# Huguet57/LIMO-Velo

Measured on AMD Instinct MI355X. Metric: KF-update iters/sec, 64k-pt scan vs 1M-pt map, higher is better.
Workload: dtype f32 (kNN/plane fit) + f64 (Jacobian rows, H^T H, 23-dof solve)

## Files before the change

### limo-velo_amd/csrc/lv_api.hip

```cpp
#include <cmath>
#include <cstdlib>
#include <cstring>
#include <limits>
#include <new>

#include "lv_filter.hpp"
#include "lv_host.hpp"
#include "lv_rebuild.hpp"
#include "lv_visibility.hpp"
#include "lv_paint.hpp"
#include "lv_place.hpp"

#include <chrono>

namespace lv {

static thread_local char g_err[512] = "";

void set_error(const char* fmt, ...) {
    va_list ap;
    va_start(ap, fmt);
    vsnprintf(g_err, sizeof(g_err), fmt, ap);
    va_end(ap);
}
// ... 43 lines not shown
    int grid = 1;
    bool fold_direct = false;
    bool tile_lpt = true;
    float4* d_qrec = nullptr;
    uint32_t qstride = 0;
    double* d_cpart[2] = {nullptr, nullptr};
    RankExchange ranks;
    uint32_t* d_wgcost[2] = {nullptr, nullptr};
    int pass_max_wg = 256;
    bool fused_pass = true;
    bool record_dump = false;
    bool last_update_fused = false;
    long long* d_pclk = nullptr;
    int pclk_wg = 0;
    bool keeper_by_cost = true;
    int fused_multi_round = -1;
    bool fused_ext = true;

    bool capture = false;
    size_t cap_n = 0;
    DebugOut dbg{};
    bool dbg_valid = false;
    bool qrec_valid = false;

    bool begin_pending = false;
    BeginArg h_begin;
    int fallback_base = 0;
    long mailbox_resyncs = 0;

    int pass_index = -1;
    bool coll_timed = false;
    bool fast_fit = false;
    bool multi_overlap = true;
    bool in_update = false;
    bool want_log = false;
    int passes_issued = 0;

    bool profiling = false;
    bool phase_clocks = false;
    long long* d_clk = nullptr;
    hipEvent_t ev_begin = nullptr, ev_end = nullptr;
    std::vector<hipEvent_t> ev_pass;
    hipEvent_t ev_mid = nullptr;
    std::vector<hipEvent_t> ev_coll;
    lv_timing timing{};
};

namespace {

struct SlowCall {
    const char* name;
    std::chrono::steady_clock::time_point t0;
    static double limit_ms() { static const double v = [] { const char* e = getenv("LV_SLOW_CALL_MS"); return e ? atof(e) : 0.0; }(); return v; }
    explicit SlowCall(const char* n) : name(n) { if (limit_ms() > 0.0) t0 = std::chrono::steady_clock::now(); }
    ~SlowCall() {
        if (limit_ms() > 0.0) {
            const double ms = std::chrono::duration<double, std::milli>(std::chrono::steady_clock::now() - t0).count();
            if (ms > limit_ms()) fprintf(stderr, "[limovelo_hip] slow call: %s took %.3f ms\n", name, ms);
        }
    }
};
#define LV_CHECK_CTX(ctx)                        \
    SlowCall _slow_call(__func__);               \
    do {                                         \
        if (!(ctx)) {                            \
            set_error("null context");           \
// ... 80 lines not shown
                const double theta = (A[q][q] - A[p][p]) / (2.0 * apq);
                const double t = (theta >= 0.0 ? 1.0 : -1.0) / (std::fabs(theta) + std::sqrt(theta * theta + 1.0));
                const double c = 1.0 / std::sqrt(t * t + 1.0), s = t * c;
                for (int k = 0; k < 6; ++k) {
                    const double akp = A[k][p], akq = A[k][q];
                    A[k][p] = c * akp - s * akq;
                    A[k][q] = s * akp + c * akq;
                }
                for (int k = 0; k < 6; ++k) {
                    const double apk = A[p][k], aqk = A[q][k];
                    A[p][k] = c * apk - s * aqk;
                    A[q][k] = s * apk + c * aqk;
                }
            }
    for (int i = 0; i < 6; ++i) eig[i] = A[i][i];
}

void unpack_sums(const double* rec, lv_sums* out) {
    int idx = 0;
    for (int i = 0; i < 12; ++i)
        for (int j = i; j < 12; ++j) {
            out->HTH[i * 12 + j] = rec[idx];
            out->HTH[j * 12 + i] = rec[idx];
            ++idx;
        }
    for (int i = 0; i < 12; ++i) out->HTh[i] = rec[78 + i];
    out->n_valid = (int64_t)rec[90];
    out->sum_h2 = rec[91];
}

int begin_device(lv_ctx* c, const double* x_host, bool defer, const ResidentFilter::Prior& prior = {}) {
    if (int rf = c->filter.begin_update(c->stream, c->d_kf, prior.dev != nullptr)) return rf;
    c->begin_pending = false;
    if (c->capture) LV_HIP(hipMemsetAsync(c->d_kf->level_hist, 0, sizeof(int) * 8, c->stream));
    if (defer && x_host && c->scan.n > 0 && c->map.view.m > 0) {
        std::memcpy(c->h_begin.x, x_host, sizeof(c->h_begin.x));
        std::memcpy(c->h_begin.P, x_host + NX, sizeof(c->h_begin.P));
        compute_pose_consts(c->h_begin.x, &c->h_begin.pose);
        c->begin_pending = true;
    } else {
        int rc = launch_kf_begin(c->stream, c->d_kf, c->d_io, x_host, prior.dev, prior.dev_in_kf);
        if (rc) return rc;
    }
    c->grid = fit_grid_size(c->scan.n, c->max_blocks);
    if ((uint32_t)c->scan.n > c->qstride) {
        uint32_t cap = c->qstride ? c->qstride : 4096;
        while (cap < (uint32_t)c->scan.n) cap *= 2;
        LV_HIP(hipStreamSynchronize(c->stream));
        hipFree(c->d_qrec);
        c->d_qrec = nullptr;
        c->qstride = 0;
        LV_HIP(hipMalloc(&c->d_qrec, (size_t)cap * qrec_slots(c->prm.NUM_MATCH_POINTS) * sizeof(float4)));
        c->qstride = cap;
    }
    return LV_OK;
}

int begin_common(lv_ctx* c, const lv_state* x, const double* P, bool defer = true) {
    KfHostIO* io = c->h_io;
    std::memcpy(io->x_in, x, sizeof(double) * NX);
    if (P) {
        std::memcpy(io->P_in, P, sizeof(double) * NS * NS);
    } else {
        for (int i = 0; i < NS * NS; ++i) io->P_in[i] = (i / NS == i % NS) ? 1.0 : 0.0;
    }
    c->update_seq = (c->update_seq + 1) & 0x3fffffff;
    return begin_device(c, io->x_in, defer);
// ... 92 lines not shown
    if (c->ranks.multi_rank() && !c->ranks.fits((size_t)nwg * partial_width(c))) return false;
    return c->fused_pass && !c->capture && !c->phase_clocks && c->prm.degeneracy_mode <= 1 && c->prm.NUM_MATCH_POINTS == KNN &&
           c->prm.lanes_per_query == 8 && (c->prm.estimate_extrinsics == 0 || c->fused_ext) && c->map.view.m > 0;
}

int update_fused(lv_ctx* c) {
    const int npass = c->prm.MAX_NUM_ITERS + 1;
    PassLaunch pl{};
    pl.map = &c->map.view;
    pl.scan = c->scan.d_sorted;
    pl.tile_order = (c->tile_lpt && c->scan.tile_points == 32u && c->scan.n_tiles == (c->scan.n + 31u) / 32u) ? c->scan.d_tile_order : nullptr;
    pl.n = c->scan.n;
    pl.kf = c->d_kf;
    pl.io = c->d_io;
    pl.sums_out = c->d_sums;
    pl.mp.R_inv = 1.0 / c->prm.LiDAR_noise;
    pl.mp.max_dist_plane_sq = c->prm.MAX_DIST_PLANE * c->prm.MAX_DIST_PLANE;
    pl.mp.planes_threshold = c->prm.PLANES_THRESHOLD;
    pl.mp.estimate_extrinsics = c->prm.estimate_extrinsics;
    pl.mp.fast_fit = c->fast_fit && !c->prm.estimate_extrinsics;
    pl.sp.R = c->prm.LiDAR_noise;
    pl.sp.R_inv = 1.0 / c->prm.LiDAR_noise;
    for (int i = 0; i < NS; ++i) pl.sp.limits[i] = c->prm.LIMITS[i];
    pl.sp.maximum_iter = c->prm.MAX_NUM_ITERS;
    pl.sp.estimate_extrinsics = c->prm.estimate_extrinsics;
    pl.sp.seq = c->update_seq;
    pl.sp.degeneracy_mode = 0;
    pl.sp.degeneracy_threshold = c->prm.degeneracy_threshold;
    int nwg = 0, rounds = 0, steps = 0, dedicated = 0;
    pass_grid_size(pass_geometry_points(c), c->pass_max_wg, &nwg, &steps, &rounds, &dedicated);
    const bool gathered = c->ranks.multi_rank();
    const size_t slot = (size_t)nwg * partial_width(c);
    pl.multi_overlap = c->multi_overlap;
    pl.qrec = c->record_dump ? c->d_qrec : nullptr;
    c->pclk_wg = nwg + dedicated;
    pl.qstride = c->qstride;
    c->qrec_valid = c->record_dump;
    c->last_update_fused = true;
    for (int i = 0; i <= npass; ++i) {
        const bool closing = i == npass;
        pl.mode = i == 0 ? (c->begin_pending ? 0 : 2) : 1;
        pl.recs_in = gathered ? c->ranks.d_gather[(i + 1) & 1] : c->d_cpart[(i + 1) & 1];
        pl.part_out = gathered ? c->ranks.part_out(i & 1, slot) : c->d_cpart[i & 1];
        pl.nrec = c->ranks.nrec(nwg);
        pl.cost_in = (i > 0 && c->keeper_by_cost) ? c->d_wgcost[(i + 1) & 1] : nullptr;
        pl.cost_out = c->d_wgcost[i & 1];
        pl.nwg = nwg;
        pl.rounds = closing ? 0 : rounds;
        pl.steps = steps;
        pl.dedicated = dedicated;
        pl.launch = i;
        pl.clk = c->d_pclk ? c->d_pclk + (size_t)i * (c->pass_max_wg + 1) * pass_clock_words() : nullptr;
        if (c->profiling && !closing) LV_HIP(hipEventRecord(c->ev_pass[3 * i + 0], c->stream));
        int rc = launch_pass(c->stream, pl, (i == 0 && c->begin_pending) ? &c->h_begin : nullptr);
        c->begin_pending = false;
        if (rc) return rc;
        if (c->profiling && !closing) LV_HIP(hipEventRecord(c->ev_pass[3 * i + 1], c->stream));
        if (gathered && !closing) {
            if (c->profiling) LV_HIP(hipEventRecord(c->ev_coll[2 * i], c->stream));
            if ((rc = c->ranks.exchange(c->stream, i, slot))) return rc;
            if (c->profiling) LV_HIP(hipEventRecord(c->ev_coll[2 * i + 1], c->stream));
        }
        if (c->profiling && !closing) LV_HIP(hipEventRecord(c->ev_pass[3 * i + 2], c->stream));
    }
    c->coll_timed = gathered && c->profiling;
    return LV_OK;
}

}

extern "C" {

void lv_default_params(lv_params* p) {
    if (!p) return;
    std::memset(p, 0, sizeof(*p));
    p->MAX_NUM_ITERS = 3;
    p->NUM_MATCH_POINTS = 5;
    p->MAX_DIST_PLANE = 2.0;
    p->PLANES_THRESHOLD = 5.e-2f;
// ... 31 lines not shown
        if (!warned) {
            warned = true;
            fprintf(stderr, "limovelo_hip: degeneracy_threshold = %g is set but has no effect: the degeneracy stage of the fork's "
                            "update_iterated_dyn_share_modified is not part of the reference mount; degeneracy_mode = 2 enables a "
                            "documented restatement, degeneracy_mode = 1 reports the eigenvalues (include/limovelo_hip.h)\n",
                    params->degeneracy_threshold);
        }
    }
    int ndev = 0;
    hipError_t e = hipGetDeviceCount(&ndev);
    if (e != hipSuccess || ndev <= 0) { set_error("no HIP device available (%s)", hipGetErrorString(e)); return LV_ENODEV; }
    if (device < 0 || device >= ndev) { set_error("device %d out of range (%d devices)", device, ndev); return LV_EINVAL; }
    LV_HIP(hipSetDevice(device));
    lv_ctx* c = new (std::nothrow) lv_ctx();
    if (!c) { set_error("out of host memory"); return LV_EINVAL; }
    c->prm = *params;
    c->device = device;
    c->scan.tile_points = 256u / (uint32_t)S;
    c->map.cell = params->voxel_size;
    hipDeviceProp_t prop;
    LV_HIP(hipGetDeviceProperties(&prop, device));
    int per_cu = 4;
    if (const char* e = getenv("LV_BLOCKS_PER_CU")) per_cu = atoi(e) > 0 ? atoi(e) : 4;
    if (const char* e = getenv("LV_TILE_LPT")) c->tile_lpt = atoi(e) != 0;
    if (const char* e = getenv("LV_SPIN_WAIT")) c->spin_wait = atoi(e) != 0;
    if (const char* e = getenv("LV_FUSED_PASS")) c->fused_pass = atoi(e) != 0;
    if (const char* e = getenv("LV_FUSED_EXT")) c->fused_ext = atoi(e) != 0;
    if (const char* e = getenv("LV_FUSED_MULTI")) c->fused_multi_round = atoi(e) != 0 ? 1 : 0;
    if (const char* e = getenv("LV_ASYNC_RELINEARISE")) c->rebuild.opt.async = atoi(e) != 0;
    if (const char* e = getenv("LV_RELIN_SLICE_WGS")) c->rebuild.opt.slice_wgs = (uint32_t)atol(e);
    if (const char* e = getenv("LV_RELIN_PAUSE_US")) c->rebuild.opt.pause_us = (uint32_t)atol(e);
    if (const char* e = getenv("LV_MULTI_OVERLAP")) c->multi_overlap = atoi(e) != 0;
    if (const char* e = getenv("LV_KEEPER_BY_COST")) c->keeper_by_cost = atoi(e) != 0;
    if (const char* e = getenv("LV_COMM_FUSED")) c->ranks.fused = atoi(e) != 0;
    if (const char* e = getenv("LV_SMALL_WINDOW")) c->scan.small_enabled = atoi(e) != 0;
    if (const char* e = getenv("LV_LARGE_WINDOW")) c->scan.large_enabled = atoi(e) != 0;
    if (const char* e = getenv("LV_MAIL_FILTER")) c->filter.mail_filter = atoi(e) != 0;
    if (const char* e = getenv("LV_SMALL_INSERT")) c->map.small_front = atoi(e) != 0;
    if (const char* e = getenv("LV_SURV_LIST")) c->map.surv_list = atoi(e) != 0;
    c->pass_max_wg = prop.multiProcessorCount;
    if (const char* e = getenv("LV_PASS_WG")) c->pass_max_wg = atoi(e) > 0 ? atoi(e) : c->pass_max_wg;
    if (const char* e = getenv("LV_PASS_CLK")) {
        if (atoi(e) != 0) {
            const size_t words = (size_t)(MAX_PASSES + 1) * (c->pass_max_wg + 1) * pass_clock_words();
            LV_HIP(hipMalloc(&c->d_pclk, words * sizeof(long long)));
            LV_HIP(hipMemset(c->d_pclk, 0, words * sizeof(long long)));
        }
    }
    c->max_blocks = prop.multiProcessorCount * per_cu;
    if (c->max_blocks < 64) c->max_blocks = 64;
    LV_HIP(hipStreamCreateWithFlags(&c->own_stream, hipStreamNonBlocking));
    c->stream = c->own_stream;
    LV_HIP(hipStreamCreateWithFlags(&c->side_stream, hipStreamNonBlocking));
    c->rebuild.create_streams(device, true);
    LV_HIP(hipEventCreateWithFlags(&c->ev_staged, hipEventDisableTiming));
    if (const char* e = getenv("LV_OVERLAP_INSERT")) c->overlap_insert = atoi(e) != 0;
    if (const char* e = getenv("LV_BATCH_PREDICT")) c->filter.batch_predict = atoi(e) != 0;
    if (const char* e = getenv("LV_MERGED_INSERT")) c->map.merged_back = atoi(e) != 0;
    if (const char* e = getenv("LV_SWEEP_EVICT")) c->map.sweep_evict = atoi(e) != 0;
    LV_HIP(hipMalloc(&c->d_kf, sizeof(KfDev)));
    LV_HIP(hipMemset(c->d_kf, 0, sizeof(KfDev)));
    if (int rf = c->filter.alloc()) return rf;
    LV_HIP(hipHostMalloc((void**)&c->h_kf, sizeof(KfDev), hipHostMallocDefault));
    std::memset(c->h_kf, 0, sizeof(KfDev));
    LV_HIP(hipHostMalloc((void**)&c->h_io, sizeof(KfHostIO), hipHostMallocMapped));
    std::memset(c->h_io, 0, sizeof(KfHostIO));
// ... 981 lines not shown
}

int lv_last_update_fused(lv_ctx* c) { return (c && c->last_update_fused) ? 1 : 0; }
int lv_last_passes(lv_ctx* c) { return c ? c->h_io->passes : 0; }

int lv_pass_geometry(size_t n_scan, int n_cus, int out[4]) {
    if (!out || n_cus < 1 || n_scan > 0xFFFFFFF0ull) { set_error("lv_pass_geometry: bad arguments"); return LV_EINVAL; }
    pass_grid_size((uint32_t)n_scan, n_cus, &out[0], &out[1], &out[2], &out[3]);
    return LV_OK;
}

int lv_set_fused_pass(lv_ctx* c, int enabled) {
    LV_CHECK_CTX(c);
    c->fused_pass = enabled != 0;
    return LV_OK;
}

int lv_set_option(lv_ctx* c, const char* name, int value) {
    LV_CHECK_CTX(c);
    if (!name) { set_error("null argument"); return LV_EINVAL; }
    if (c->in_update) { set_error("lv_set_option inside an update"); return LV_ESTATE; }
    const bool on = value != 0;
    if (!std::strcmp(name, "fused_pass")) c->fused_pass = on;
    else if (!std::strcmp(name, "fused_ext")) c->fused_ext = on;
    else if (!std::strcmp(name, "fast_fit")) c->fast_fit = on;
    else if (!std::strcmp(name, "async_relinearise")) c->rebuild.opt.async = on;
    else if (!std::strcmp(name, "async_relinearise_min")) c->rebuild.opt.async_min = value > 0 ? (size_t)value : 0;
    else if (!std::strcmp(name, "async_relinearise_pause_us")) c->rebuild.opt.pause_us = value > 0 ? (uint32_t)value : 0u;
    else if (!std::strcmp(name, "async_relinearise_slice_wgs")) c->rebuild.opt.slice_wgs = value > 0 ? (uint32_t)value : 0u;
    else if (!std::strcmp(name, "async_relinearise_journal_max")) c->rebuild.opt.journal_max = value > 0 ? (size_t)value : 1;
    else if (!std::strcmp(name, "async_relinearise_test_delay_ms")) c->rebuild.opt.test_delay_ms = value;
    else if (!std::strcmp(name, "async_relinearise_test_race")) c->rebuild.opt.test_race = on;
    else if (!std::strcmp(name, "multi_overlap")) c->multi_overlap = on;
    else if (!std::strcmp(name, "fused_multi_round")) c->fused_multi_round = on ? 1 : 0;
    else if (!std::strcmp(name, "keeper_by_cost")) c->keeper_by_cost = on;
    else if (!std::strcmp(name, "tile_lpt")) c->tile_lpt = on;
    else if (!std::strcmp(name, "spin_wait")) c->spin_wait = on;
    else if (!std::strcmp(name, "comm_fused")) c->ranks.fused = on;
    else if (!std::strcmp(name, "mail_filter")) c->filter.mail_filter = on;
    else if (!std::strcmp(name, "overlap_insert")) c->overlap_insert = on;
    else if (!std::strcmp(name, "batch_predict")) { if (int rp = c->filter.flush(c->stream, c->d_kf)) return rp; c->filter.batch_predict = on; }
    else if (!std::strcmp(name, "merged_insert")) c->map.merged_back = on;
    else if (!std::strcmp(name, "sweep_evict")) c->map.sweep_evict = on;
    else if (!std::strcmp(name, "small_window")) c->scan.small_enabled = on;
    else if (!std::strcmp(name, "large_window")) c->scan.large_enabled = on;
    else if (!std::strcmp(name, "small_insert")) c->map.small_front = on;
    else if (!std::strcmp(name, "survivor_list")) c->map.surv_list = on;
    else if (!std::strcmp(name, "batch_chunk_hypotheses")) c->batch.chunk_hyp = value > 0 ? value : 0;
    else { set_error("lv_set_option: unknown option '%s'", name); return LV_EINVAL; }
    return LV_OK;
}

int lv_get_pass_clocks(lv_ctx* c, long long* out, int capacity_wg, int* n_wg) {
    LV_CHECK_CTX(c);
    if (!c->d_pclk) { set_error("no pass clocks: create the context with LV_PASS_CLK=1 in the environment"); return LV_ESTATE; }
    const int slots = c->pass_max_wg + 1;
    if (!out) {
        if (n_wg) *n_wg = slots;
        return LV_OK;
    }
    if (capacity_wg < slots) { set_error("lv_get_pass_clocks: capacity %d < %d workgroup slots per launch", capacity_wg, slots); return LV_EINVAL; }
    LV_HIP(hipStreamSynchronize(c->stream));
    LV_HIP(hipMemcpy(out, c->d_pclk, (size_t)(c->prm.MAX_NUM_ITERS + 2) * slots * pass_clock_words() * sizeof(long long), hipMemcpyDeviceToHost));
    if (n_wg) *n_wg = c->pclk_wg;
    return LV_OK;
}
// ... 463 lines not shown
```

### limo-velo_amd/csrc/lv_host.hpp

```cpp
#pragma once
#include "lv_note.hpp"

#include <cstdarg>
#include <cstdio>
#include <vector>

#include "../../include/limovelo_hip.h"
#include "lv_device.hpp"
#include "lv_common.hpp"
#include "lv_exchange.hpp"
#include "lv_mapinc.hpp"

namespace lv {

struct MapStats {
    uint64_t living, ids, capacity;
    uint64_t pool_used[4], pool_cap[4];
    uint64_t slots_used[4], slots_cap[4];
    uint64_t tombstones, dropped;
    uint64_t relinearisations, incremental_adds;
    uint64_t bytes;
};

struct MapStore {
// ... 188 lines not shown
int launch_kf_begin(hipStream_t stream, KfDev* kf, KfHostIO* io, const double* x_host, const FilterDev* filt = nullptr, int filt_in_kf = 0);
int launch_reduce_groups(hipStream_t stream, const double* partials, int nblocks, double* groups, int* ngroups_out, KfDev* kf);
int solve_direct_records();
int launch_reduce_final(hipStream_t stream, const double* groups, int ngroups, double* sums, KfDev* kf);
struct SolveParams {
    double R;
    double R_inv;
    double limits[NS];
    int maximum_iter;
    int estimate_extrinsics;
    int seq;
    int degeneracy_mode;
    double degeneracy_threshold;
};
int launch_solve(hipStream_t stream, KfDev* kf, KfHostIO* io, const double* recs, int nrec, double* sums_out, const SolveParams& prm);
struct PassLaunch {
    const MapView* map;
    const float4* scan;
    const uint32_t* tile_order;
    uint32_t n;
    KfDev* kf;
    KfHostIO* io;
    const double* recs_in;
    double* part_out;
    double* sums_out;
    float4* qrec;
    long long* clk;
    uint32_t qstride;
    int nrec;
    int mode;
    int rounds, launch, nwg;
    const uint32_t* cost_in;
    uint32_t* cost_out;
    bool multi_overlap = true;
    int steps, dedicated;
    MatchParams mp;
    SolveParams sp;
};
void pass_grid_size(uint32_t n, int max_wg, int* nsearch, int* steps, int* rounds, int* dedicated);
constexpr int PK_DEFAULT_MAX_ROUNDS = 16;
int pass_clock_words();
int launch_pass(hipStream_t stream, const PassLaunch& pl, const BeginArg* begin);
int launch_filter_to_kf(hipStream_t stream, const FilterDev* f, KfDev* kf);
int launch_rows_from_matches(hipStream_t stream, const KfDev* kf, const float* p_world, const float* abcd, const float* dist,
                             uint32_t n, int estimate_extrinsics, double* H, double* h);
struct CloudPoint;
struct ScanStore {
    float4* d_raw = nullptr;
    float4* d_sorted = nullptr;
    uint32_t* d_keys = nullptr;
    uint32_t* d_keys_sorted = nullptr;
    uint32_t* d_idx = nullptr;
    uint32_t* d_idx_sorted = nullptr;
    void* d_sort_tmp = nullptr;
    size_t sort_tmp_bytes = 0;
    size_t capacity = 0;
    uint32_t n = 0;
    uint32_t* d_tile_order = nullptr;
    uint32_t n_tiles = 0, tile_cap = 0;
    uint32_t tile_points = 0;
    float4* d_in = nullptr;
    double* d_times = nullptr;
    float4* d_desk = nullptr;
    MotionState* d_states = nullptr;
    uint64_t* d_vkeys = nullptr;
    uint64_t* d_vkeys_sorted = nullptr;
    uint32_t* d_vidx = nullptr;
    uint32_t* d_vidx_sorted = nullptr;
    uint32_t* d_heads = nullptr;
    uint32_t* d_hpos = nullptr;
    unsigned* d_bounds = nullptr;
    void* d_vsort_tmp = nullptr;
    void* d_vscan_tmp = nullptr;
// ... 84 lines not shown
```

### limo-velo_amd/csrc/lv_match.hip

```cpp
#include "lv_host.hpp"
#include "lv_pass_dev.hpp"

#ifndef LV_HALF_CHUNK
#define LV_HALF_CHUNK 1
#endif
#ifndef LV_QR_SELECT
#define LV_QR_SELECT 1
#endif
#include "lv_search_dev.hpp"

namespace lv {

__device__ __forceinline__ void sort8(kkey (&c)[8]) {
    cswap(c[0], c[1]); cswap(c[2], c[3]); cswap(c[4], c[5]); cswap(c[6], c[7]);
    cswap(c[0], c[2]); cswap(c[1], c[3]); cswap(c[4], c[6]); cswap(c[5], c[7]);
    cswap(c[1], c[2]); cswap(c[5], c[6]);
    cswap(c[0], c[4]); cswap(c[1], c[5]); cswap(c[2], c[6]); cswap(c[3], c[7]);
    cswap(c[2], c[4]); cswap(c[3], c[5]);
    cswap(c[1], c[2]); cswap(c[3], c[4]); cswap(c[5], c[6]);
}
__device__ __forceinline__ void order_unimodal5(kkey (&c)[5]) {
    cswap(c[0], c[4]); cswap(c[1], c[3]); cswap(c[1], c[4]); cswap(c[2], c[4]); cswap(c[3], c[4]);
}
template <int K>
// ... 530 lines not shown
                if (lane == 0) atomicAdd(&kf->fallback_queries, 1);
                done = cells_attempt(map, ((wgeo.c0x >> 3) - 1) * 2, ((wgeo.c0y >> 3) - 1) * 2, ((wgeo.c0z >> 3) - 1) * 2, 6, search_radius(map, wgeo, 3),
                                     wx, wy, wz, lane, kw, s_pref, s_start);
                if (done) wbin = 3;
            }
        } else {
            float r = search_radius(map, wgeo, 2);
            int side = 3, bx = c2x - 1, by = c2y - 1, bz = c2z - 1;
            if (!(r > 0.f && (double)(r * r) >= max_dist_sq)) {
                side = 4;
                bx = c2x - 1 - ((wgeo.tx - (float)((c2x << 2) - CELL_OFFSET)) < 2.f ? 1 : 0);
                by = c2y - 1 - ((wgeo.ty - (float)((c2y << 2) - CELL_OFFSET)) < 2.f ? 1 : 0);
                bz = c2z - 1 - ((wgeo.tz - (float)((c2z << 2) - CELL_OFFSET)) < 2.f ? 1 : 0);
                r = block_radius(map, wgeo, 2, bx, by, bz, 4);
                if (lane == 0) atomicAdd(&kf->fallback_queries, 1);
            }
            done = cells_attempt(map, bx, by, bz, side, r, wx, wy, wz, lane, kw, s_pref, s_start, &wgeo, bound);
            if (done) wbin = side == 3 ? 2 : 3;
            stop = r > 0.f && (double)(r * r) >= max_dist_sq;
        }
        if (!done && !stop) { brute_attempt(map, wx, wy, wz, lane, kw); wbin = 4; }
    } else {
        if (lane == 0) atomicAdd(&kf->fallback_queries, 1);
        brute_attempt(map, wx, wy, wz, lane, kw);
        wbin = 4;
    }
    return wbin;
}

template <int S, bool DBG, int K>
__device__ __forceinline__ void knn_search(const MapView& map, KfDev* __restrict__ kf, float qx, float qy, float qz, int gl,
                                           kkey (&k)[K], uint32_t& bstart, int& src, long long* clk, bool hist,
                                           bool live, Xyz* stage0, double max_dist_sq, uint32_t* s_pref, uint32_t* s_start,
                                           bool* undecided = nullptr, uint32_t* bound_out = nullptr) {
    if (undecided) *undecided = false;
    if (map.m == 0) return;
    const QGeom geo = make_geom(map, qx, qy, qz);
    const bool finite = __builtin_isfinite(qx) && __builtin_isfinite(qy) && __builtin_isfinite(qz);
    const bool in_range = finite && geo.amax < CELL_FAR;
    bool decided = !live || !finite;
    int hist_bin = -1;
    uint32_t bound = 0x7FFFFFFFu;
    if (live && in_range) {
#pragma unroll
#ifndef LV_DIAG_LEVELS
#define LV_DIAG_LEVELS 2
#endif
        for (int bl = 0; bl < LV_DIAG_LEVELS; ++bl) {
            if (!decided) {
                decided = bucket_attempt<S>(map, bl, geo, qx, qy, qz, gl, k, bstart, (DBG && bl == 0) ? clk : nullptr,
                                            bl == 0 ? stage0 : nullptr, bl == 1 ? &bound : nullptr);
                if (decided) { src = bl; hist_bin = bl; }
            }
        }
    }
    if (undecided) {
        *undecided = !decided;
        if (bound_out) *bound_out = bound;
        return;
    }
    const int lane = (int)(threadIdx.x & 63u);
    unsigned long long pending = __ballot(!decided && gl == 0);
    while (pending) {
        const int L = __ffsll((long long)pending) - 1;
        pending &= pending - 1;
        const float wx = __shfl(qx, L), wy = __shfl(qy, L), wz = __shfl(qz, L);
        const uint32_t wbound = (uint32_t)__shfl((int)bound, L);
        kkey kw[K];
        const int wbin = knn_coarse<DBG>(map, kf, wx, wy, wz, lane, kw, max_dist_sq, s_pref, s_start, wbound);
        if (lane / S == L / S) {
#pragma unroll
            for (int j = 0; j < K; ++j) k[j] = kw[j];
            hist_bin = wbin;
            decided = true;
        }
    }
    if (DBG && hist && live && finite && gl == 0) atomicAdd(&kf->level_hist[hist_bin >= 0 ? hist_bin : 5], 1);
}

template <int W, bool EXT, bool DBG, int K, bool KEEP = false, bool FAST = false>
__device__ __forceinline__ void fit_row(const PoseConsts& pc, const MatchParams& prm, const DebugOut& dbg, int found,
                                        const float (&P)[K][3], const uint32_t (&nidx)[K], const uint32_t (&dbits)[K],
                                        float qx, float qy, float qz, uint32_t oq, double* srow, double* keep = nullptr) {
    double row[W];
// ... 367 lines not shown
        case 3: LV_LAUNCH_K(3); break;
        case 4: LV_LAUNCH_K(4); break;
        case KNN: LV_LAUNCH_K(KNN); break;
        case 6: LV_LAUNCH_K(6); break;
        case 7: LV_LAUNCH_K(7); break;
        case 8: LV_LAUNCH_K(8); break;
        default: set_error("NUM_MATCH_POINTS must be 3..8 (got %d)", num_match); return LV_EINVAL;
    }
#undef LV_LAUNCH_K
#undef LV_LAUNCH
    LV_HIP(hipGetLastError());
    return LV_OK;
}


struct PassArgs {
    MapView map;
    const float4* scan;
    const uint32_t* tile_order;
    uint32_t n, n_tiles32;
    KfDev* kf;
    KfHostIO* io;
    const double* recs_in;
    double* part_out;
    double* sums_out;
    float4* qrec;
    long long* clk;
    uint32_t qstride;
    int nrec, mode, rounds, launch;
    const uint32_t* cost_in;
    uint32_t* cost_out;
    int steps;
    uint32_t nsearch;
    MatchParams mp;
    SolveParams sp;
};
constexpr int PK_UNITS = PK_THREADS / 256;
constexpr int PK_GROUPS = PK_THREADS / 8;
constexpr int PK_STAGE = 64;
constexpr int PK_STEPS = 2048 / PK_THREADS;
constexpr int PK_FITW = PK_STEPS * PK_GROUPS / 64;
constexpr int PK_RPTS_MAX = PK_STEPS * PK_GROUPS;
constexpr int PK_CLK = 32;
constexpr size_t PK_REGION0 = sizeof(Xyz) * PK_GROUPS * PK_STAGE < 65536 ? 65536 : sizeof(Xyz) * PK_GROUPS * PK_STAGE;
constexpr size_t PK_OFF_REC = PK_REGION0;
constexpr size_t PK_OFF_PREF = PK_OFF_REC + sizeof(float4) * PK_STEPS * QREC_SLOTS * PK_GROUPS;
constexpr size_t PK_OFF_POSE = PK_OFF_PREF + sizeof(uint32_t) * 2 * (PK_THREADS / 64) * 64;
constexpr size_t PK_OFF_OUT = PK_OFF_POSE + ((sizeof(PoseConsts) + 15) / 16) * 16;
constexpr size_t PK_OFF_KEEP = PK_OFF_OUT + sizeof(double) * PK_FITW * 2 * SUMS_LEN;
constexpr size_t PK_OFF_QN = PK_OFF_KEEP + ((sizeof(KeepLds) + 15) / 16) * 16;
constexpr size_t PK_OFF_QUEUE = PK_OFF_QN + 32;
constexpr size_t PK_OFF_QUEUEQ = PK_OFF_QUEUE + sizeof(float4) * PK_RPTS_MAX;
constexpr size_t PK_OFF_QUEUEB = PK_OFF_QUEUEQ + sizeof(uint32_t) * PK_RPTS_MAX;
constexpr size_t PK_LDS_BYTES = PK_OFF_QUEUEB + sizeof(uint32_t) * PK_RPTS_MAX;
constexpr size_t PK_OFF_BOOK = 32 * 1024;
static_assert(sizeof(SolveLds) <= PK_OFF_BOOK && PK_OFF_BOOK + sizeof(BookLds) <= PK_REGION0, "solve / books scratch must fit under the stage");
static_assert(sizeof(double) * PK_FITW * 64 * 14 <= PK_OFF_BOOK, "staged rows must stay below the books' scratch");
static_assert(PK_LDS_BYTES <= 160 * 1024, "one workgroup per CU");

template <int W, int T, class Bar>
__device__ __forceinline__ void keeper_books(const PassArgs& a, const BeginArg& begin, KeepLds& K, BookLds& Bk, KfDev* __restrict__ kf,
                                             const KfDev::PassState* __restrict__ ps_in, KfDev::PassState* __restrict__ ps_out,
                                             const PoseConsts* pose, int tid, Bar& bar, long long* clk) {
    if (a.mode == 1) {
        bookkeeping<W, T>(K, Bk, kf, ps_in, ps_out, a.io, a.sums_out, a.sp.R_inv, a.sp.seq, pose, K.Pprop, K.xp, false, tid, bar, clk);
        return;
// ... 51 lines not shown
    constexpr int W = EXT ? 12 : 6;
    constexpr int ROW_W = W + 2;
    constexpr int NOUT = PassDims<W>::NOUT, OW = PassDims<W>::OW;
    constexpr int NACC = (NOUT + 63) / 64;
    constexpr bool HALVES = NOUT <= 32;
    __shared__ __attribute__((aligned(16))) unsigned char smem[PK_LDS_BYTES];
    SolveLds& L = *reinterpret_cast<SolveLds*>(smem);
    BookLds& Bk = *reinterpret_cast<BookLds*>(smem + PK_OFF_BOOK);
    Xyz (*s_stage)[PK_STAGE] = reinterpret_cast<Xyz (*)[PK_STAGE]>(smem);
    constexpr bool TWO_PHASE = MULTI && EXT;
    constexpr int ROWS_STAGED = TWO_PHASE ? 32 : 64;
    constexpr size_t ROWS_STRIDE = MULTI ? sizeof(Xyz) * 8 * PK_STAGE : sizeof(double) * 64 * ROW_W;
    static_assert(sizeof(double) * ROWS_STAGED * ROW_W <= ROWS_STRIDE && ROWS_STRIDE * PK_FITW <= PK_OFF_BOOK, "staged rows: inside the stride, below the books");
    float4* s_rec = reinterpret_cast<float4*>(smem + PK_OFF_REC);
    uint32_t (*s_pref)[64] = reinterpret_cast<uint32_t (*)[64]>(smem + PK_OFF_PREF);
    uint32_t (*s_start)[64] = s_pref + PK_THREADS / 64;
    PoseConsts& s_pose = *reinterpret_cast<PoseConsts*>(smem + PK_OFF_POSE);
    double (*s_out)[2][SUMS_LEN] = reinterpret_cast<double (*)[2][SUMS_LEN]>(smem + PK_OFF_OUT);

    const int tid = threadIdx.x;
    const int wave = tid >> 6, lane = tid & 63;
    const uint32_t nwg = a.nsearch, bid = blockIdx.x;
    const bool dedicated = gridDim.x > nwg;
    bool keeper = bid == gridDim.x - 1u;
    const long long t_begin = wall_clock64();
    KfDev* __restrict__ kf = a.kf;
    const KfDev::PassState* __restrict__ ps_in = &kf->ps[a.launch & 1];
    KfDev::PassState* __restrict__ ps_out = &kf->ps[(a.launch + 1) & 1];
    KeepLds& K = *reinterpret_cast<KeepLds*>(smem + PK_OFF_KEEP);
    int* s_qn = reinterpret_cast<int*>(smem + PK_OFF_QN);
    float4* s_queue = reinterpret_cast<float4*>(smem + PK_OFF_QUEUE);
    uint32_t* s_queueq = reinterpret_cast<uint32_t*>(smem + PK_OFF_QUEUEQ);
    uint32_t* s_queueb = reinterpret_cast<uint32_t*>(smem + PK_OFF_QUEUEB);
    if (threadIdx.x < 8) s_qn[threadIdx.x] = 0;
    bool books_done = false;
    constexpr int NW32 = (int)(sizeof(PoseConsts) / 4);
    long long* clk = a.clk ? a.clk + (size_t)bid * PK_CLK : nullptr;
#define PK_STAMP(i, cond) do { if (clk && (cond)) { clk[i] = clock64(); clk[16 + (i)] = wall_clock64(); } } while (0)
    PK_STAMP(0, tid == 0);
    if (clk && tid == 0) clk[16 + 10] = 0;

    const bool searching = !CLOSING && a.rounds > 0 && bid < nwg;
    if (a.mode == 1) {
        if (CLOSING) {
            for (int e = tid; e < NS * NS; e += PK_THREADS) Bk.P[e / NS][e % NS] = ps_in->prep_P[e];
            if (tid < NX) Bk.xp[tid] = kf->x_prop[tid];
            set_identity<PK_THREADS>(Bk.J, tid);
        }
        const bool choose = !CLOSING && !dedicated && a.cost_in != nullptr;
        if (!solve_core<W, !CLOSING>(L, kf, ps_in, a.recs_in, a.nrec, a.sp, &s_pose, tid, clk, choose ? a.cost_in : nullptr, choose ? (int)nwg : 0,
                                     CLOSING ? &Bk : nullptr))
            return;
        if (choose && L.cheapest >= 0) keeper = (int)bid == L.cheapest;
        if (keeper) {
            keep_solve(K, L, tid);
            if (!CLOSING) {
                for (int e = tid; e < NS * NS; e += PK_THREADS) K.Pprop[e] = kf->P_prop[e];
                if (tid < NX) K.xp[tid] = kf->x_prop[tid];
            }
        }
        const int ended = L.last;
        __syncthreads();
        if (ended || !searching) {
            if (!keeper) return;
            WgBar bar;
            const bool closing = a.rounds == 0;
            bookkeeping<W, PK_THREADS>(K, Bk, kf, ps_in, ps_out, a.io, a.sums_out, a.sp.R_inv, a.sp.seq, &s_pose, closing ? kf->P_prop : K.Pprop,
                                       closing ? kf->x_prop : K.xp, closing, tid, bar, clk, CLOSING);
            PK_STAMP(10, tid == 0);
            return;
        }
    } else {
        if (a.mode == 2 && kf->done) return;
        if (tid < NW32)
            reinterpret_cast<uint32_t*>(&s_pose)[tid] =
                a.mode == 0 ? reinterpret_cast<const uint32_t*>(&begin.pose)[tid] : reinterpret_cast<const uint32_t*>(&kf->pose)[tid];
        __syncthreads();
    }
    PK_STAMP(3, tid == 0);

    if constexpr (!CLOSING) {
    if (searching) {
    const int gq = tid / S, gl = tid % S;
    const int fstep = wave / (PK_GROUPS / 64), fbase = (wave % (PK_GROUPS / 64)) * 64;
    const bool fitter = wave < PK_FITW && fstep < a.steps;
    int oa[NACC], ob[NACC];
    double acc[NACC];
    const int olane = HALVES ? (lane & 31) : lane;
    const int prow0 = HALVES ? (lane >> 5) * 32 : 0;
#pragma unroll
    for (int c = 0; c < NACC; ++c) {
        int orec_unused = 0;
        oa[c] = ob[c] = 0;
        acc[c] = 0.0;
        if (olane + c * 64 < NOUT) out_pair<W>(olane + c * 64, oa[c], ob[c], orec_unused);
    }
    for (int t = tid; t < PK_FITW * 2 * SUMS_LEN; t += PK_THREADS) (&s_out[0][0][0])[t] = 0.0;
    const DebugOut nodbg{};
    auto do_fits = [&](bool stamp, bool release_records) __attribute__((always_inline)) {
        const float4* rec = s_rec + (size_t)fstep * QREC_SLOTS * PK_GROUPS + fbase;
        float4 r[QREC_SLOTS];
#pragma unroll
        for (int sl = 0; sl < QREC_SLOTS; ++sl) r[sl] = rec[sl * PK_GROUPS + lane];
        if (release_records) {
            __builtin_amdgcn_fence(__ATOMIC_RELEASE, "workgroup");
            if (lane == 0) atomicAdd(s_qn + 5, 1);
        }
        float P[KNN][3];
        uint32_t nidx[KNN], dbits[KNN];
#pragma unroll
        for (int j = 0; j < KNN; ++j) { P[j][0] = r[j].x; P[j][1] = r[j].y; P[j][2] = r[j].z; nidx[j] = __float_as_uint(r[j].w); }
        dbits[0] = __float_as_uint(r[6].x); dbits[1] = __float_as_uint(r[6].y); dbits[2] = __float_as_uint(r[6].z);
        dbits[3] = __float_as_uint(r[6].w); dbits[4] = __float_as_uint(r[7].x);
        const int found = __float_as_int(r[7].y);
        double (*rows_w)[ROW_W] = reinterpret_cast<double (*)[ROW_W]>(smem + (size_t)wave * ROWS_STRIDE);
        const double (*rows)[ROW_W] = rows_w;
        if constexpr (TWO_PHASE) {
            double keep[ROW_W];
            fit_row<W, EXT, false, KNN, true>(s_pose, a.mp, nodbg, found, P, nidx, dbits, r[5].x, r[5].y, r[5].z, __float_as_uint(r[5].w), nullptr, keep);
#pragma unroll
            for (int half = 0; half < 2; ++half) {
                if ((lane >> 5) == half) {
#pragma unroll
                    for (int j = 0; j < ROW_W; ++j) rows_w[lane & 31][j] = keep[j];
                }
                wave_lds_fence();
                if (stamp && half == 1) PK_STAMP(7, tid == 0);
#pragma unroll
                for (int c = 0; c < NACC; ++c) {
                    if (olane + c * 64 < NOUT) {
                        double sacc = acc[c];
#pragma unroll 8
// ... 30 lines not shown
            task = __builtin_amdgcn_readfirstlane(task);
            if (task >= ntask) break;
            if (MULTI && round > 0) {
                const int want = a.steps * (PK_GROUPS / 64) * round;
                int spin = 0;
                for (; spin < (1 << 20) && __hip_atomic_load(s_qn + 5, __ATOMIC_ACQUIRE, __HIP_MEMORY_SCOPE_WORKGROUP) < want; ++spin)
                    __builtin_amdgcn_s_sleep(1);
                if (spin == (1 << 20) && lane == 0) atomicOr(reinterpret_cast<unsigned int*>(&kf->fallback_queries), KF_FAULT_BIT);
            }
            const int step = task / (PK_THREADS / 64);
            const int gqv = (task % (PK_THREADS / 64)) * 8 + (lane >> 3);
            const uint32_t band = (uint32_t)((round * a.steps + step) * PK_UNITS + (gqv >> 5));
            const uint32_t vbi = band * nwg + ((band & 1u) ? nwg - 1u - bid : bid);
            const bool tile_ok = vbi < a.n_tiles32;
            float4* rec = s_rec + (size_t)step * QREC_SLOTS * PK_GROUPS;
            if (!tile_ok) {
                if (gl == 7) rec[7 * PK_GROUPS + gqv] = make_float4(0.f, __int_as_float(-1), 0.f, 0.f);
                continue;
            }
            const uint32_t tile = a.tile_order ? a.tile_order[vbi] : vbi;
            const uint32_t q = tile * 32u + (uint32_t)(gqv & 31);
            const bool live = q < a.n;
            kkey k[KNN];
#pragma unroll
            for (int j = 0; j < KNN; ++j) k[j] = none_key();
            uint32_t bstart = 0;
            int src = -1;
            const float4 sp = a.scan[live ? q : a.n - 1];
            float qx, qy, qz;
            rt_apply(s_pose.Tc, sp.x, sp.y, sp.z, qx, qy, qz);
            bool open_pt = false;
            uint32_t open_bound = 0x7FFFFFFFu;
            knn_search<S, false>(a.map, kf, qx, qy, qz, gl, k, bstart, src, nullptr, false, live, s_stage[gq], a.mp.max_dist_plane_sq,
                                 s_pref[wave], s_start[wave], &open_pt, &open_bound);
            if (open_pt && gl == 0) {
                const int qi = atomicAdd(s_qcnt, 1);
                s_queue[qi] = make_float4(qx, qy, qz, __int_as_float(step * PK_GROUPS + gqv));
                s_queueq[qi] = q;
                s_queueb[qi] = open_bound;
            }
            int found = 0;
#pragma unroll
            for (int j = 0; j < KNN; ++j) found += key_real(k[j]) ? 1 : 0;
            {
                const int slot = gl;
                float4 v;
                if (slot < KNN) {
                    kkey kk = k[0];
#pragma unroll
                    for (int j = 1; j < KNN; ++j) kk = (slot == j) ? k[j] : kk;
                    v = make_float4(0.f, 0.f, 0.f, __uint_as_float(0xFFFFFFFFu));
                    if (live && key_real(kk)) {
                        const uint32_t pos = key_lo(kk);
                        if (src == 0 && pos < (uint32_t)PK_STAGE) {
                            const Xyz w = s_stage[gq][pos];
                            v = make_float4(w.x, w.y, w.z, __uint_as_float(0xFFFFFFFFu));
                        } else if (src >= 0) {
                            const Xyz w = reinterpret_cast<const Xyz*>(a.map.bxyz[0])[(size_t)bstart + pos];
                            v = make_float4(w.x, w.y, w.z, __uint_as_float(0xFFFFFFFFu));
                        } else {
                            v = a.map.orig[pos];
                            v.w = __uint_as_float(pos);
                        }
                    }
                } else if (slot == 5) {
                    v = make_float4(qx, qy, qz, sp.w);
                } else if (slot == 6) {
// ... 37 lines not shown
                        kkey kk = kw[0];
#pragma unroll
                        for (int j = 1; j < KNN; ++j) kk = (slot == j) ? kw[j] : kk;
                        v = make_float4(0.f, 0.f, 0.f, __uint_as_float(0xFFFFFFFFu));
                        if (key_real(kk)) {
                            const uint32_t pos = key_lo(kk);
                            v = a.map.orig[pos];
                            v.w = __uint_as_float(pos);
                        }
                    } else if (slot == 6) {
                        v = make_float4(__uint_as_float(key_hi(kw[0])), __uint_as_float(key_hi(kw[1])), __uint_as_float(key_hi(kw[2])),
                                        __uint_as_float(key_hi(kw[3])));
                    } else {
                        v = make_float4(__uint_as_float(key_hi(kw[4])), __int_as_float(found), 0.f, 0.f);
                    }
                    s_rec[((p / PK_GROUPS) * QREC_SLOTS + slot) * PK_GROUPS + (p % PK_GROUPS)] = v;
                    if (a.qrec) a.qrec[(size_t)slot * a.qstride + q] = v;
                }
            }
            __syncthreads();
            if (tid == 0) *s_qcnt = 0;
        }
        if (round + 1 < a.rounds) {
            if constexpr (!MULTI) {
                if (fitter) do_fits(false, false);
                __syncthreads();
            } else if (fitter) {
                do_fits(false, true);
            }
        }
    }
    {
        const bool beside = a.mode == 1 && keeper && 64 * PK_BOOKW >= NS * W;
        if (fitter) {
            do_fits(true, false);
        } else if (beside && wave >= PK_FITW) {
            SubBar bar(s_qn + 2, PK_BOOKW);
            bookkeeping<W, 64 * PK_BOOKW>(K, Bk, kf, ps_in, ps_out, a.io, a.sums_out, a.sp.R_inv, a.sp.seq, &s_pose, K.Pprop, K.xp, false,
                                          tid - 64 * PK_FITW, bar, clk);
            PK_STAMP(10, tid == 64 * PK_FITW);
        }
        books_done = beside;
        PK_STAMP(8, tid == 0);
        __syncthreads();
    }
    if (fitter) {
#pragma unroll
        for (int c = 0; c < NACC; ++c)
            if (olane + c * 64 < NOUT) s_out[wave][HALVES ? (lane >> 5) : 0][olane + c * 64] = acc[c];
    }
    __syncthreads();
    if (tid < OW) {
        double s = 0.0;
        if (tid < NOUT) {
            s = s_out[0][0][tid] + s_out[0][1][tid];
#pragma unroll
            for (int f = 1; f < PK_FITW; ++f) s += s_out[f][0][tid] + s_out[f][1][tid];
        }
        a.part_out[(size_t)bid * OW + tid] = s;
    }
    }
    if (a.cost_out && tid == 0 && bid < nwg) a.cost_out[bid] = (uint32_t)(wall_clock64() - t_begin);
    }
    PK_STAMP(9, tid == 0);
    if (!keeper || books_done) return;
    {
        WgBar bar;
        keeper_books<W, PK_THREADS>(a, begin, K, Bk, kf, ps_in, ps_out, &s_pose, tid, bar, clk);
    }
    PK_STAMP(10, tid == 0);
#undef PK_STAMP
}

void pass_grid_size(uint32_t n, int max_wg, int* nsearch, int* steps, int* rounds, int* dedicated) {
    const uint32_t nt = (n + 31u) / 32u, U = (uint32_t)PK_UNITS, M = (uint32_t)(max_wg > 1 ? max_wg : 2);
    uint32_t st, g;
    if (nt <= U * M) { st = 1; g = (nt + U - 1u) / U; }
    else { st = (uint32_t)PK_STEPS; g = (nt + st * U - 1u) / (st * U); }
    const bool ded = g <= M - 1u;
    if (g > M) g = M;
    if (g < 1) g = 1;
    static const bool split = [] { const char* e = getenv("LV_PASS_SPLIT"); return e && atoi(e) != 0; }();
    if (split && st == (uint32_t)PK_STEPS && (nt + st * U * g - 1u) / (st * U * g) == 1u && nt > U * g) st = 1;
    *nsearch = (int)g;
    *steps = (int)st;
    *rounds = (int)((nt + st * U * g - 1u) / (st * U * g));
    *dedicated = ded ? 1 : 0;
}
int pass_clock_words() { return PK_CLK; }

int launch_pass(hipStream_t stream, const PassLaunch& pl, const BeginArg* begin) {
    PassArgs a;
    a.map = *pl.map;
    a.scan = pl.scan;
    a.tile_order = pl.tile_order;
    a.n = pl.n;
    a.n_tiles32 = (pl.n + 31u) / 32u;
    a.kf = pl.kf;
    a.io = pl.io;
    a.recs_in = pl.recs_in;
    a.part_out = pl.part_out;
    a.sums_out = pl.sums_out;
    a.qrec = pl.qrec;
    a.clk = pl.clk;
    a.qstride = pl.qstride;
    a.nrec = pl.nrec;
    a.mode = pl.mode;
    a.rounds = pl.rounds;
    a.launch = pl.launch;
    a.steps = pl.steps;
    a.cost_in = pl.cost_in;
    a.cost_out = pl.cost_out;
    a.nsearch = (uint32_t)pl.nwg;
    a.mp = pl.mp;
    a.sp = pl.sp;
    static const BeginArg none{};
    const BeginArg& b = begin ? *begin : none;
    const dim3 grid((unsigned)(pl.rounds > 0 ? pl.nwg + (pl.dedicated ? 1 : 0) : 1)), block(PK_THREADS);
    const bool closing = pl.rounds == 0;
    if (pl.mp.estimate_extrinsics) {
        if (closing) hipLaunchKernelGGL((pass_kernel<true, true>), grid, block, 0, stream, a, b);
        else if (pl.rounds > 1 && pl.multi_overlap) hipLaunchKernelGGL((pass_kernel<true, false, true>), grid, block, 0, stream, a, b);
        else hipLaunchKernelGGL((pass_kernel<true, false>), grid, block, 0, stream, a, b);
    } else {
        if (closing) hipLaunchKernelGGL((pass_kernel<false, true>), grid, block, 0, stream, a, b);
        else if (pl.rounds > 1 && pl.multi_overlap) {
            if (pl.mp.fast_fit) hipLaunchKernelGGL((pass_kernel<false, false, true, true>), grid, block, 0, stream, a, b);
            else hipLaunchKernelGGL((pass_kernel<false, false, true>), grid, block, 0, stream, a, b);
        } else {
            if (pl.mp.fast_fit) hipLaunchKernelGGL((pass_kernel<false, false, false, true>), grid, block, 0, stream, a, b);
            else hipLaunchKernelGGL((pass_kernel<false, false>), grid, block, 0, stream, a, b);
        }
    }
    LV_HIP(hipGetLastError());
    return LV_OK;
}

#endif

}
```

Measured before the change: 28760.

## Skip level-1 bucket attempt per workgroup when prior pass saw few open queries

Each workgroup counts queries left undecided or resolved at bucket level 1 and writes that count into a spare slot of its partial-sum record. On the next pass the workgroup reads its own count, and if it is below a threshold (default 128) it enters a sparse mode that skips the level-1 bucket attempt. Those queries go straight to the open-point queue, with the level-0 bound used instead. The aim is to cut redundant level-1 probing when few points need it, at the cost of more queued fallback work and an extra cross-pass feedback dependency.

```diff
diff --git a/limo-velo_amd/csrc/lv_api.hip b/limo-velo_amd/csrc/lv_api.hip
--- a/limo-velo_amd/csrc/lv_api.hip
+++ b/limo-velo_amd/csrc/lv_api.hip
@@ -99,6 +99,7 @@
     bool coll_timed = false;
     bool fast_fit = false;
     bool multi_overlap = true;
+    int sparse_level1_max = LV_SPARSE_LEVEL1_DEFAULT;
     bool in_update = false;
     bool want_log = false;
     int passes_issued = 0;
@@ -245,7 +246,7 @@
 int begin_device(lv_ctx* c, const double* x_host, bool defer, const ResidentFilter::Prior& prior = {}) {
     if (int rf = c->filter.begin_update(c->stream, c->d_kf, prior.dev != nullptr)) return rf;
     c->begin_pending = false;
-    if (c->capture) LV_HIP(hipMemsetAsync(c->d_kf->level_hist, 0, sizeof(int) * 8, c->stream));
+    if (c->capture) LV_HIP(hipMemsetAsync(c->d_kf->level_hist, 0, sizeof(int) * 6, c->stream));
     if (defer && x_host && c->scan.n > 0 && c->map.view.m > 0) {
         std::memcpy(c->h_begin.x, x_host, sizeof(c->h_begin.x));
         std::memcpy(c->h_begin.P, x_host + NX, sizeof(c->h_begin.P));
@@ -404,7 +405,9 @@
     const bool gathered = c->ranks.multi_rank();
     const size_t slot = (size_t)nwg * partial_width(c);
     pl.multi_overlap = c->multi_overlap;
-    pl.qrec = c->record_dump ? c->d_qrec : nullptr;
+    pl.sparse_max = gathered ? 0 : c->sparse_level1_max;
+    pl.sparse_first = (steps == 1 && rounds == 1) || (long long)pl.sparse_max >= 256LL * rounds;
+    pl.qrec =c->record_dump ? c->d_qrec : nullptr;
     c->pclk_wg = nwg + dedicated;
     pl.qstride = c->qstride;
     c->qrec_valid = c->record_dump;
@@ -417,6 +420,7 @@
         pl.nrec = c->ranks.nrec(nwg);
         pl.cost_in = (i > 0 && c->keeper_by_cost) ? c->d_wgcost[(i + 1) & 1] : nullptr;
         pl.cost_out = c->d_wgcost[i & 1];
+        pl.open_in = (i > 0 && !gathered) ? c->d_cpart[(i + 1) & 1] : nullptr;
         pl.nwg = nwg;
         pl.rounds = closing ? 0 : rounds;
         pl.steps = steps;
@@ -514,6 +518,7 @@
     if (const char* e = getenv("LV_RELIN_PAUSE_US")) c->rebuild.opt.pause_us = (uint32_t)atol(e);
     if (const char* e = getenv("LV_MULTI_OVERLAP")) c->multi_overlap = atoi(e) != 0;
     if (const char* e = getenv("LV_KEEPER_BY_COST")) c->keeper_by_cost = atoi(e) != 0;
+    if (const char* e = getenv("LV_SPARSE_LEVEL1_MAX")) c->sparse_level1_max = atoi(e) > 0 ? atoi(e) : 0;
     if (const char* e = getenv("LV_COMM_FUSED")) c->ranks.fused = atoi(e) != 0;
     if (const char* e = getenv("LV_SMALL_WINDOW")) c->scan.small_enabled = atoi(e) != 0;
     if (const char* e = getenv("LV_LARGE_WINDOW")) c->scan.large_enabled = atoi(e) != 0;
@@ -1561,6 +1566,7 @@
     else if (!std::strcmp(name, "async_relinearise_test_delay_ms")) c->rebuild.opt.test_delay_ms = value;
     else if (!std::strcmp(name, "async_relinearise_test_race")) c->rebuild.opt.test_race = on;
     else if (!std::strcmp(name, "multi_overlap")) c->multi_overlap = on;
+    else if (!std::strcmp(name, "sparse_level1_max")) c->sparse_level1_max = value > 0 ? value : 0;
     else if (!std::strcmp(name, "fused_multi_round")) c->fused_multi_round = on ? 1 : 0;
     else if (!std::strcmp(name, "keeper_by_cost")) c->keeper_by_cost = on;
     else if (!std::strcmp(name, "tile_lpt")) c->tile_lpt = on;
diff --git a/limo-velo_amd/csrc/lv_host.hpp b/limo-velo_amd/csrc/lv_host.hpp
--- a/limo-velo_amd/csrc/lv_host.hpp
+++ b/limo-velo_amd/csrc/lv_host.hpp
@@ -244,6 +244,9 @@
     int rounds, launch, nwg;
     const uint32_t* cost_in;
     uint32_t* cost_out;
+    const double* open_in = nullptr;
+    int sparse_max = 0;
+    bool sparse_first = false;
     bool multi_overlap = true;
     int steps, dedicated;
     MatchParams mp;
@@ -251,6 +254,9 @@
 };
 void pass_grid_size(uint32_t n, int max_wg, int* nsearch, int* steps, int* rounds, int* dedicated);
 constexpr int PK_DEFAULT_MAX_ROUNDS = 16;
+#ifndef LV_SPARSE_LEVEL1_DEFAULT
+#define LV_SPARSE_LEVEL1_DEFAULT 128
+#endif
 int pass_clock_words();
 int launch_pass(hipStream_t stream, const PassLaunch& pl, const BeginArg* begin);
 int launch_filter_to_kf(hipStream_t stream, const FilterDev* f, KfDev* kf);
diff --git a/limo-velo_amd/csrc/lv_match.hip b/limo-velo_amd/csrc/lv_match.hip
--- a/limo-velo_amd/csrc/lv_match.hip
+++ b/limo-velo_amd/csrc/lv_match.hip
@@ -586,7 +586,7 @@
 __device__ __forceinline__ void knn_search(const MapView& map, KfDev* __restrict__ kf, float qx, float qy, float qz, int gl,
                                            kkey (&k)[K], uint32_t& bstart, int& src, long long* clk, bool hist,
                                            bool live, Xyz* stage0, double max_dist_sq, uint32_t* s_pref, uint32_t* s_start,
-                                           bool* undecided = nullptr, uint32_t* bound_out = nullptr) {
+                                           bool* undecided = nullptr, uint32_t* bound_out = nullptr, bool sparse = false) {
     if (undecided) *undecided = false;
     if (map.m == 0) return;
     const QGeom geo = make_geom(map, qx, qy, qz);
@@ -601,9 +601,9 @@
 #define LV_DIAG_LEVELS 2
 #endif
         for (int bl = 0; bl < LV_DIAG_LEVELS; ++bl) {
-            if (!decided) {
+            if (!decided && !(bl == 1 && sparse)) {
                 decided = bucket_attempt<S>(map, bl, geo, qx, qy, qz, gl, k, bstart, (DBG && bl == 0) ? clk : nullptr,
-                                            bl == 0 ? stage0 : nullptr, bl == 1 ? &bound : nullptr);
+                                            bl == 0 ? stage0 : nullptr, (bl == 1 || sparse) ? &bound : nullptr);
                 if (decided) { src = bl; hist_bin = bl; }
             }
         }
@@ -1037,6 +1037,8 @@
     uint32_t* cost_out;
     int steps;
     uint32_t nsearch;
+    const double* open_in;
+    int sparse_max, sparse_first;
     MatchParams mp;
     SolveParams sp;
 };
@@ -1154,7 +1156,14 @@
     float4* s_queue = reinterpret_cast<float4*>(smem + PK_OFF_QUEUE);
     uint32_t* s_queueq = reinterpret_cast<uint32_t*>(smem + PK_OFF_QUEUEQ);
     uint32_t* s_queueb = reinterpret_cast<uint32_t*>(smem + PK_OFF_QUEUEB);
-    if (threadIdx.x < 8) s_qn[threadIdx.x] = 0;
+    if (threadIdx.x < 8) {
+        int v = 0;
+        if (!CLOSING && threadIdx.x == 7) {
+            if (a.mode != 1) v = a.sparse_first;
+            else if (a.open_in && blockIdx.x < a.nsearch) v = a.open_in[(size_t)blockIdx.x * OW + NOUT] <= (double)a.sparse_max ? 1 : 0;
+        }
+        s_qn[threadIdx.x] = v;
+    }
     bool books_done = false;
     constexpr int NW32 = (int)(sizeof(PoseConsts) / 4);
     long long* clk = a.clk ? a.clk + (size_t)bid * PK_CLK : nullptr;
@@ -1219,7 +1228,9 @@
     }
     for (int t = tid; t < PK_FITW * 2 * SUMS_LEN; t += PK_THREADS) (&s_out[0][0][0])[t] = 0.0;
     const DebugOut nodbg{};
-    auto do_fits = [&](bool stamp, bool release_records) __attribute__((always_inline)) {
+    const bool sparse = __builtin_amdgcn_readfirstlane(s_qn[7]) != 0;
+    int nopen = 0;
+    auto do_fits =[&](bool stamp, bool release_records) __attribute__((always_inline)) {
         const float4* rec = s_rec + (size_t)fstep * QREC_SLOTS * PK_GROUPS + fbase;
         float4 r[QREC_SLOTS];
 #pragma unroll
@@ -1316,7 +1327,8 @@
             bool open_pt = false;
             uint32_t open_bound = 0x7FFFFFFFu;
             knn_search<S, false>(a.map, kf, qx, qy, qz, gl, k, bstart, src, nullptr, false, live, s_stage[gq], a.mp.max_dist_plane_sq,
-                                 s_pref[wave], s_start[wave], &open_pt, &open_bound);
+                                 s_pref[wave], s_start[wave], &open_pt, &open_bound, sparse);
+            nopen += __popcll(__ballot(gl == 0 && (open_pt || src == 1)));
             if (open_pt && gl == 0) {
                 const int qi = atomicAdd(s_qcnt, 1);
                 s_queue[qi] = make_float4(qx, qy, qz, __int_as_float(step * PK_GROUPS + gqv));
@@ -1420,6 +1432,7 @@
     }
     {
         const bool beside = a.mode == 1 && keeper && 64 * PK_BOOKW >= NS * W;
+        if (lane == 0 && nopen) atomicAdd(s_qn + 6, nopen);
         if (fitter) {
             do_fits(true, false);
         } else if (beside && wave >= PK_FITW) {
@@ -1444,6 +1457,10 @@
             s = s_out[0][0][tid] + s_out[0][1][tid];
 #pragma unroll
             for (int f = 1; f < PK_FITW; ++f) s += s_out[f][0][tid] + s_out[f][1][tid];
+        } else if (tid == NOUT) {
+            const int cnt = s_qn[6];
+            s = (double)cnt;
+            if (cnt) atomicAdd(&kf->level_hist[sparse ? 6 : 7], cnt);
         }
         a.part_out[(size_t)bid * OW + tid] = s;
     }
@@ -1500,6 +1517,9 @@
     a.cost_in = pl.cost_in;
     a.cost_out = pl.cost_out;
     a.nsearch = (uint32_t)pl.nwg;
+    a.open_in = pl.sparse_max > 0 ? pl.open_in : nullptr;
+    a.sparse_max = pl.sparse_max;
+    a.sparse_first = pl.sparse_max > 0 && pl.sparse_first ? 1 : 0;
     a.mp = pl.mp;
     a.sp = pl.sp;
     static const BeginArg none{};
```

New measurement: 27790, median of 2. 3.4% lower.
